# FREDZEL2020/jittor-MYC-NeRFs

Measured on AMD Instinct MI355X. Metric: ray_samples_per_sec, higher is better.
Workload: dtype f32 (emulated: 3 x f16-split MFMA products, fp32 accumulate; fp32 VALU elsewhere); 1 GPU; TensorVMSplit 300^3 (16/48 comps, MLP_Fea 150-128-128-3), 800x800 rays x 512 samples/ray (BASELINE configs[1]); ONE frame per step at every N (N>1: split over the ranks, BASELINE configs[2]), 512-ray tiles round-robin, one RCCL all_gather of [4 cap] fp32 (rgb block + depth block, written in place by the render) + two strided un-permute copies; scene=synthetic scene A (SURVEY 8d), no alpha mask, white_bg, samples_per_ray=512, rays_per_rank=640000, tile=512, chunk=640000, alpha_mask=0, emulate_world=0, arith=f32

## Files before the change

jittor-myc-nerfs_amd/csrc/tvr_march.hip:

```cpp
#include <cstdlib>
#include "tvr_device.h"
#include "tvr_kernels.h"
#include "tvr_march_body.h"
#include "tvr_gradient.h"


template <bool DENSE, bool LDSL>
__global__ __launch_bounds__(64 * MARCH_MAX_WAVES) void march_kernel(const SceneDev sc, const float *__restrict__ rays,
                                                                     const int n_rays, const int S, const int s_cap,
                                                                     const MarchSampling sm, const float eps_T,
                                                                     MarchOut mo, const tvr_dense_out dn)
{
    constexpr bool CP = false, VOL = false;
    const CpDev cp = {};
    const float *const dvol = nullptr;
#include "tvr_march_body.inc"
}

template <bool DENSE>
__global__ __launch_bounds__(64 * MARCH_VOL_WAVES, DENSE ? MARCH_VOL_OCC - 1 : MARCH_VOL_OCC) void march_vol_kernel(const SceneDev sc, const float *__restrict__ dvol, const float *__restrict__ rays,
                                                                         const int n_rays, const int S, const int s_cap, const MarchSampling sm, const float eps_T,
                                                                         MarchOut mo, const tvr_dense_out dn)
{
    constexpr bool LDSL = false, CP = false, VOL = true;
    const CpDev cp = {};
#include "tvr_march_body.inc"
}

__global__ __launch_bounds__(256) void density_volume_kernel(const SceneDev sc, float *__restrict__ out)
{
    const long long gx1 = sc.grid[0] + 1, gy1 = sc.grid[1] + 1, gz1 = sc.grid[2] + 1;
    const long long t = (long long)blockIdx.x * blockDim.x + threadIdx.x;
    if (t >= gx1 * gy1 * gz1) return;
    const long long x = t % gx1, y = (t / gx1) % gy1, z = t / (gx1 * gy1);
    const float4 *P[3] = {sc.dplane[0] + (y * gx1 + x) * 4, sc.dplane[1] + (z * gx1 + x) * 4, sc.dplane[2] + (z * gy1 + y) * 4};
    const float4 *Ln[3] = {sc.dline[0] + z * 4, sc.dline[1] + y * 4, sc.dline[2] + x * 4};
    double acc = 0.0;
#pragma unroll
    for (int i = 0; i < 3; ++i) {
#pragma unroll
        for (int g = 0; g < 4; ++g) {
            const float4 p = P[i][g], l = Ln[i][g];
            acc = acc + (double)p.x * (double)l.x;
            acc = acc + (double)p.y * (double)l.y;
            acc = acc + (double)p.z * (double)l.z;
            acc = acc + (double)p.w * (double)l.w;
        }
    }
    out[t] = (float)acc;
}

hipError_t launch_density_volume(const SceneDev &sc, float *out, hipStream_t stream)
{
    const long long n = ((long long)sc.grid[0] + 1) * ((long long)sc.grid[1] + 1) * ((long long)sc.grid[2] + 1);
    hipLaunchKernelGGL(density_volume_kernel, dim3((unsigned)((n + 255) / 256)), dim3(256), 0, stream, sc, out);
    return hipGetLastError();
}

#define COMP_LANES 8
__global__ __launch_bounds__(256) void composite_kernel(const MarchOut mo, const int n_rays, const int white_bg,
                                                        float *__restrict__ rgb_out)
{
    const int t = blockIdx.x * blockDim.x + threadIdx.x;
    const int r = t / COMP_LANES, l = t % COMP_LANES;
    const bool live = r < n_rays;
    const unsigned base = live ? mo.ray_off[r] : 0u, cnt = live ? mo.ray_cnt[r] : 0u;
    float c0 = 0.f, c1 = 0.f, c2 = 0.f;
    unsigned i = l;
    for (; i + 3 * COMP_LANES < cnt; i += 4 * COMP_LANES) {
        const float4 e0 = mo.q_out[base + i], e1 = mo.q_out[base + i + COMP_LANES], e2 = mo.q_out[base + i + 2 * COMP_LANES],
                     e3 = mo.q_out[base + i + 3 * COMP_LANES];
        c0 = c0 + e0.w * e0.x; c1 = c1 + e0.w * e0.y; c2 = c2 + e0.w * e0.z;
        c0 = c0 + e1.w * e1.x; c1 = c1 + e1.w * e1.y; c2 = c2 + e1.w * e1.z;
        c0 = c0 + e2.w * e2.x; c1 = c1 + e2.w * e2.y; c2 = c2 + e2.w * e2.z;
        c0 = c0 + e3.w * e3.x; c1 = c1 + e3.w * e3.y; c2 = c2 + e3.w * e3.z;
    }
    for (; i < cnt; i += COMP_LANES) {
        const float4 e = mo.q_out[base + i];
        c0 = c0 + e.w * e.x;
        c1 = c1 + e.w * e.y;
        c2 = c2 + e.w * e.z;
    }
#pragma unroll
    for (int off = 1; off < COMP_LANES; off <<= 1) {
        c0 = c0 + __shfl_xor(c0, off);
        c1 = c1 + __shfl_xor(c1, off);
        c2 = c2 + __shfl_xor(c2, off);
    }
    if (!live || l != 0) return;
    if (mo.counter[2] != 0u) {
        const float qnan = __int_as_float(0x7fc00000);
        rgb_out[(size_t)r * 3 + 0] = qnan; rgb_out[(size_t)r * 3 + 1] = qnan; rgb_out[(size_t)r * 3 + 2] = qnan;
        mo.depth[r] = qnan;
        return;
    }
    const float acc = mo.acc[r];
    if (white_bg) {
        const float bg = 1.0f - acc;
        c0 = c0 + bg; c1 = c1 + bg; c2 = c2 + bg;
    }
    rgb_out[(size_t)r * 3 + 0] = clamp01(c0);
    rgb_out[(size_t)r * 3 + 1] = clamp01(c1);
    rgb_out[(size_t)r * 3 + 2] = clamp01(c2);
}

__global__ __launch_bounds__(256) void scatter_rgb_kernel(const MarchOut mo, const int S, float *__restrict__ rgb_dense)
{
    const unsigned n = *mo.counter;
    for (unsigned e = blockIdx.x * blockDim.x + threadIdx.x; e < n; e += gridDim.x * blockDim.x) {
        const float4 v = mo.q_out[e];
        const size_t q = ((size_t)mo.q_ray[e] * S + mo.q_j[e]) * 3;
        rgb_dense[q] = v.x; rgb_dense[q + 1] = v.y; rgb_dense[q + 2] = v.z;
    }
}

__global__ __launch_bounds__(256) void density_feature_kernel(const SceneDev sc, const float *__restrict__ xyz, const long long m,
                                                              float *__restrict__ out)
{
    const long long t = (long long)blockIdx.x * blockDim.x + threadIdx.x;
    const long long s = t >> 2;
    const int sub = threadIdx.x & 3;
    float part = 0.0f;
    if (s < m) {
        int i0[3];
        float w[3];
#pragma unroll
        for (int k = 0; k < 3; ++k) {
            const float f = unnorm(xyz[s * 3 + k], sc.gm1[k]);
            const float fl = floorf(fminf(fmaxf(f, -2.0f), sc.gm1[k] + 2.0f));
            i0[k] = (int)fl;
            w[k] = f - fl;
        }
        const float4 a = vm_term<4, true>(sc.dplane[0], sc.dline[0], sc.grid[0], sc.grid[1], sc.grid[2], i0[0], i0[1], i0[2], w[0], w[1], w[2], sub);
        const float4 b = vm_term<4, true>(sc.dplane[1], sc.dline[1], sc.grid[0], sc.grid[2], sc.grid[1], i0[0], i0[2], i0[1], w[0], w[2], w[1], sub);
        const float4 c = vm_term<4, true>(sc.dplane[2], sc.dline[2], sc.grid[1], sc.grid[2], sc.grid[0], i0[1], i0[2], i0[0], w[1], w[2], w[0], sub);
        part = ((a.x + a.y) + (a.z + a.w)) + ((b.x + b.y) + (b.z + b.w)) + ((c.x + c.y) + (c.z + c.w));
    }
    part += __shfl_xor(part, 1);
    part += __shfl_xor(part, 2);
    if (s < m && sub == 0) out[s] = part;
}

__global__ __launch_bounds__(256) void density_gradient_kernel(const SceneDev sc, const float *__restrict__ xyz, const long long m, const float3 h, const float3 inv2h,
                                                               float *__restrict__ sigma_feature, float *__restrict__ grad)
{
    const long long t = (long long)blockIdx.x * blockDim.x + threadIdx.x;
    const long long s = t >> 2;
    const int sub = threadIdx.x & 3;
    float f[7];
#pragma unroll
    for (int j = 0; j < 7; ++j) f[j] = 0.0f;
    if (s < m) vm_grad_point(sc, xyz[s * 3], xyz[s * 3 + 1], xyz[s * 3 + 2], h, sub, f);
#pragma unroll
    for (int j = 0; j < 7; ++j) {
        f[j] += __shfl_xor(f[j], 1);
        f[j] += __shfl_xor(f[j], 2);
    }
    if (s < m && sub == 0) {
        if (sigma_feature) sigma_feature[s] = f[0];
        grad[s * 3 + 0] = (f[1] - f[2]) * inv2h.x;
        grad[s * 3 + 1] = (f[3] - f[4]) * inv2h.y;
        grad[s * 3 + 2] = (f[5] - f[6]) * inv2h.z;
    }
}

__global__ __launch_bounds__(256) void alpha_sample_kernel(const SceneDev sc, const float *__restrict__ xyz, const long long m,
                                                           float *__restrict__ out)
{
    const long long s = (long long)blockIdx.x * blockDim.x + threadIdx.x;
    if (s >= m) return;
    const float p[3] = {xyz[s * 3], xyz[s * 3 + 1], xyz[s * 3 + 2]};
    out[s] = alpha_lookup(sc, p);
}

__global__ __launch_bounds__(256) void alpha_bits_kernel(const float *__restrict__ vol, const long long n, unsigned *__restrict__ bits)
{
    const long long wd = (long long)blockIdx.x * blockDim.x + threadIdx.x;
    if (wd * 32 >= n) return;
    unsigned v = 0u;
    for (int b = 0; b < 32; ++b) {
        const long long i = wd * 32 + b;
        if (i < n && vol[i] > 0.0f) v |= 1u << b;
    }
    bits[wd] = v;
}

hipError_t launch_alpha_bits(const float *vol, long long n, unsigned *bits, hipStream_t stream)
{
    const long long words = (n + 31) / 32;
    hipLaunchKernelGGL(alpha_bits_kernel, dim3((unsigned)((words + 255) / 256)), dim3(256), 0, stream, vol, n, bits);
    return hipGetLastError();
}

template <bool DENSE, bool LDSL>
static hipError_t launch_march_t(const SceneDev &sc, const float *rays, int n_rays, int S, const MarchSampling &sm, float eps_T, const MarchOut &mo,
                                 const tvr_dense_out &dn, int waves, size_t lds, unsigned grid, hipStream_t stream)
{
    hipError_t rc = hipFuncSetAttribute((const void *)march_kernel<DENSE, LDSL>, hipFuncAttributeMaxDynamicSharedMemorySize, (int)lds);
    if (rc != hipSuccess) return rc;
    hipLaunchKernelGGL((march_kernel<DENSE, LDSL>), dim3(grid), dim3(64 * waves), lds, stream, sc, rays, n_rays, S, S, sm, eps_T, mo, dn);
    return hipGetLastError();
}

static int device_cu_count()
{
    static int cus = 0;
    if (cus == 0) {
        int dev = 0, n = 0;
        if (hipGetDevice(&dev) == hipSuccess && hipDeviceGetAttribute(&n, hipDeviceAttributeMultiprocessorCount, dev) == hipSuccess && n > 0) cus = n;
        else cus = 256;
    }
    return cus;
}

int march_cu_count() { return device_cu_count(); }

static hipError_t launch_march_vol(const SceneDev &sc, const float *dvol, const float *rays, int n_rays, int S, const MarchSampling &sm, float eps_T, const MarchOut &mo,
                                   const tvr_dense_out *dense, hipStream_t stream)
{
    const int groups = MARCH_VOL_GROUPS;
    const size_t kLds = 160 * 1024 / (size_t)groups, per_wave = (size_t)S * 6, fixed = MARCH_HDR + 64;
    int waves = (int)((kLds - fixed) / per_wave);
    waves = waves >= MARCH_VOL_WAVES ? MARCH_VOL_WAVES : (waves >= 8 ? 8 : (waves >= 4 ? 4 : (waves >= 2 ? 2 : 1)));
    const size_t lds = fixed + (size_t)waves * per_wave;
    const int n_tiles = (n_rays + MARCH_TILE - 1) / MARCH_TILE;
    long long grid = (long long)device_cu_count() * groups * (MARCH_VOL_WAVES / waves);
    if (grid > n_tiles) grid = n_tiles;
    if (grid < 1) grid = 1;
    tvr_dense_out none = {};
    const tvr_dense_out &dn = dense ? *dense : none;
    hipError_t rc = dense ? hipFuncSetAttribute((const void *)march_vol_kernel<true>, hipFuncAttributeMaxDynamicSharedMemorySize, (int)lds)
                          : hipFuncSetAttribute((const void *)march_vol_kernel<false>, hipFuncAttributeMaxDynamicSharedMemorySize, (int)lds);
    if (rc != hipSuccess) return rc;
    if (dense) hipLaunchKernelGGL((march_vol_kernel<true>), dim3((unsigned)grid), dim3(64 * waves), lds, stream, sc, dvol, rays, n_rays, S, S, sm, eps_T, mo, dn);
    else hipLaunchKernelGGL((march_vol_kernel<false>), dim3((unsigned)grid), dim3(64 * waves), lds, stream, sc, dvol, rays, n_rays, S, S, sm, eps_T, mo, dn);
    return hipGetLastError();
}

hipError_t launch_march(const SceneDev &sc, const float *rays, int n_rays, int S, const MarchSampling &sm, float eps_T,
                        const MarchOut &mo, const tvr_dense_out *dense, hipStream_t stream, const float *dvol)
{
    if (dvol) return launch_march_vol(sc, dvol, rays, n_rays, S, sm, eps_T, mo, dense, stream);
    const size_t kLds = 160 * 1024, line_bytes = ((size_t)sc.grid[0] + sc.grid[1] + sc.grid[2] + 3) * 16 * MARCH_LSTRIDE, per_wave = (size_t)S * 6;
    bool ldsl = MARCH_HDR + line_bytes + 4 * per_wave + 64 <= kLds;
    const size_t fixed = MARCH_HDR + (ldsl ? line_bytes : 0) + 64;
    int waves = (int)((kLds - fixed) / per_wave);
    waves = waves >= 16 ? 16 : (waves >= 12 ? 12 : (waves >= 8 ? 8 : (waves >= 4 ? 4 : (waves >= 2 ? 2 : 1))));
    const size_t lds = fixed + (size_t)waves * per_wave;
    const int n_tiles = (n_rays + MARCH_TILE - 1) / MARCH_TILE;
    long long grid = (long long)device_cu_count() * (16 / waves > 0 ? 16 / waves : 1);
    if (grid > n_tiles) grid = n_tiles;
    if (grid < 1) grid = 1;
    tvr_dense_out none = {};
    const tvr_dense_out &dn = dense ? *dense : none;
    if (dense) return ldsl ? launch_march_t<true, true>(sc, rays, n_rays, S, sm, eps_T, mo, dn, waves, lds, (unsigned)grid, stream)
                           : launch_march_t<true, false>(sc, rays, n_rays, S, sm, eps_T, mo, dn, waves, lds, (unsigned)grid, stream);
    return ldsl ? launch_march_t<false, true>(sc, rays, n_rays, S, sm, eps_T, mo, dn, waves, lds, (unsigned)grid, stream)
                : launch_march_t<false, false>(sc, rays, n_rays, S, sm, eps_T, mo, dn, waves, lds, (unsigned)grid, stream);
}

hipError_t launch_composite(const MarchOut &mo, int n_rays, int white_bg, float *rgb, hipStream_t stream)
{
    const long long threads = (long long)n_rays * COMP_LANES;
    hipLaunchKernelGGL(composite_kernel, dim3((unsigned)((threads + 255) / 256)), dim3(256), 0, stream, mo, n_rays, white_bg, rgb);
    return hipGetLastError();
}

hipError_t launch_scatter_rgb(const MarchOut &mo, int S, float *rgb_dense, hipStream_t stream)
{
    hipLaunchKernelGGL(scatter_rgb_kernel, dim3(1024), dim3(256), 0, stream, mo, S, rgb_dense);
    return hipGetLastError();
}

hipError_t launch_density_feature(const SceneDev &sc, const float *xyz, long long m, float *out, hipStream_t stream)
{
    const long long blocks = (m * 4 + 255) / 256;
    hipLaunchKernelGGL(density_feature_kernel, dim3((unsigned)blocks), dim3(256), 0, stream, sc, xyz, m, out);
    return hipGetLastError();
}

hipError_t launch_density_gradient(const SceneDev &sc, const float *xyz, long long m, const float h[3], const float inv2h[3], float *sigma_feature, float *grad,
                                   hipStream_t stream)
{
    const long long blocks = (m * 4 + 255) / 256;
    hipLaunchKernelGGL(density_gradient_kernel, dim3((unsigned)blocks), dim3(256), 0, stream, sc, xyz, m, make_float3(h[0], h[1], h[2]),
                       make_float3(inv2h[0], inv2h[1], inv2h[2]), sigma_feature, grad);
    return hipGetLastError();
}

hipError_t launch_alpha_sample(const SceneDev &sc, const float *xyz, long long m, float *out, hipStream_t stream)
{
    hipLaunchKernelGGL(alpha_sample_kernel, dim3((unsigned)((m + 255) / 256)), dim3(256), 0, stream, sc, xyz, m, out);
    return hipGetLastError();
}
```

jittor-myc-nerfs_amd/csrc/tvr_march_body.h:

```cpp
#pragma once
#include "tvr_device.h"
#include "tvr_kernels.h"

#define MARCH_MAX_WAVES 16
#define MARCH_TILE 16
#define MARCH_SPIN_LIMIT (1u << 22)
#define MARCH_SLOTS 64u
#ifndef MARCH_CTR_WORD
#define MARCH_CTR_WORD 1
#endif
#ifndef MARCH_TAIL
#define MARCH_TAIL 4u
#endif
#ifndef MARCH_VOL_WAVES
#define MARCH_VOL_WAVES 16
#endif
#ifndef MARCH_VOL_GROUPS
#define MARCH_VOL_GROUPS 1
#endif
#ifndef MARCH_VOL_OCC
#define MARCH_VOL_OCC 8
#endif
#define MARCH_HDR 560
#ifndef MARCH_LSTRIDE
#define MARCH_LSTRIDE 4
#endif

__device__ __forceinline__ float4 vm_term_lds(const float4 *__restrict__ P, const float4 *Ls, int W, int x0, int y0, int l0,
                                              float wx, float wy, float wl, int sub)
{
    const float ux = 1.0f - wx, uy = 1.0f - wy, ul = 1.0f - wl;
    const int Wp = W + 1;
    const unsigned cell = __umul24((unsigned)y0, (unsigned)Wp) + (unsigned)x0;
    unsigned o0 = (cell << 6) + ((unsigned)sub << 4), o1 = o0 + ((unsigned)Wp << 6);
    asm volatile("" : "+v"(o0), "+v"(o1));
    const unsigned char *pb = (const unsigned char *)P;
    const float4 t00 = *(const float4 *)(pb + (size_t)o0), t01 = *(const float4 *)(pb + (size_t)o0 + 64);
    const float4 t10 = *(const float4 *)(pb + (size_t)o1), t11 = *(const float4 *)(pb + (size_t)o1 + 64);
    const float4 *q = Ls + l0 * MARCH_LSTRIDE + sub;
    const float4 l0v = q[0], l1v = q[MARCH_LSTRIDE];
    float4 p4 = f4_mul(ux * uy, t00);
    p4 = f4_fma(wx * uy, t01, p4);
    p4 = f4_fma(ux * wy, t10, p4);
    p4 = f4_fma(wx * wy, t11, p4);
    float4 q4 = f4_mul(ul, l0v);
    q4 = f4_fma(wl, l1v, q4);
    return make_float4(p4.x * q4.x, p4.y * q4.y, p4.z * q4.z, p4.w * q4.w);
}

__device__ __forceinline__ float cp_density_quad(const SceneDev &sc, const CpDev &cp, int ix, int iy, int iz, float wx, float wy, float wz, int sub)
{
    const int tpt = cp.rd >> 2;
    const float4 *__restrict__ l0 = sc.dline[0] + (size_t)iz * tpt + sub;
    const float4 *__restrict__ l1 = sc.dline[1] + (size_t)iy * tpt + sub;
    const float4 *__restrict__ l2 = sc.dline[2] + (size_t)ix * tpt + sub;
    const float ux = 1.0f - wx, uy = 1.0f - wy, uz = 1.0f - wz;
    float part = 0.0f;
    for (int g = 0; g < tpt; g += 4) {
        const float4 a0 = l0[g], a1 = l0[g + tpt], b0 = l1[g], b1 = l1[g + tpt], c0 = l2[g], c1 = l2[g + tpt];
        const float4 a = f4_fma(wz, a1, f4_mul(uz, a0)), b = f4_fma(wy, b1, f4_mul(uy, b0)), c = f4_fma(wx, c1, f4_mul(ux, c0));
        const float tx = (a.x * b.x) * c.x, ty = (a.y * b.y) * c.y, tz = (a.z * b.z) * c.z, tw = (a.w * b.w) * c.w;
        part = part + ((tx + ty) + (tz + tw));
    }
    return part;
}

struct __attribute__((packed, aligned(4))) vol_pair { float a, b; };
__device__ __forceinline__ float vol_density(const float *__restrict__ D, int gx1, int gy1, int ix, int iy, int iz, float wx, float wy, float wz)
{
    const size_t sy = (size_t)gx1, sz = (size_t)gx1 * (size_t)gy1;
    const float *r = D + ((size_t)iz * sz + (size_t)iy * sy + (size_t)ix);
    const vol_pair p00 = *(const vol_pair *)r, p01 = *(const vol_pair *)(r + sy);
    const vol_pair p10 = *(const vol_pair *)(r + sz), p11 = *(const vol_pair *)(r + sz + sy);
    const float c00 = __builtin_fmaf(wx, p00.b - p00.a, p00.a), c01 = __builtin_fmaf(wx, p01.b - p01.a, p01.a);
    const float c10 = __builtin_fmaf(wx, p10.b - p10.a, p10.a), c11 = __builtin_fmaf(wx, p11.b - p11.a, p11.a);
    const float c0 = __builtin_fmaf(wy, c01 - c00, c00), c1 = __builtin_fmaf(wy, c11 - c10, c10);
    return __builtin_fmaf(wz, c1 - c0, c0);
}
```

jittor-myc-nerfs_amd/csrc/tvr_march_body.inc:

```
    static_assert(!(CP && LDSL), "the CP lines (up to 96 channels) do not go through LDS");
    static_assert(!(VOL && (CP || LDSL)), "the baked volume replaces the factored evaluation: no lines in LDS, no CP lines");
    extern __shared__ __attribute__((aligned(16))) unsigned char lds_raw[];
    const int lane = threadIdx.x & 63;
    const int wave = __builtin_amdgcn_readfirstlane(threadIdx.x >> 6);
    const int n_waves = blockDim.x >> 6;
    unsigned *cursor = (unsigned *)lds_raw;
    const float4 *ls0 = (const float4 *)(lds_raw + MARCH_HDR);
    const int ln0 = LDSL ? (sc.grid[2] + 1) * MARCH_LSTRIDE : 0, ln1 = LDSL ? (sc.grid[1] + 1) * MARCH_LSTRIDE : 0, ln2 = LDSL ? (sc.grid[0] + 1) * MARCH_LSTRIDE : 0;
    const float4 *ls1 = ls0 + ln0, *ls2 = ls1 + ln1;
    float *bufw = (float *)(ls2 + ln2) + (size_t)wave * s_cap;
    unsigned short *bufj = (unsigned short *)((float *)(ls2 + ln2) + (size_t)n_waves * s_cap) + (size_t)wave * s_cap;
#ifdef TVR_MARCH_TIMELINE
    unsigned long long tl_chunks = 0ull, tl_rays = 0ull;
    if (mo.stats && threadIdx.x == 0) mo.stats[32 + 8 * blockIdx.x] = __builtin_amdgcn_s_memrealtime();
#endif
    if (threadIdx.x == 0) *cursor = 0u;
    unsigned long long *slots = (unsigned long long *)(lds_raw + 16);
    if (threadIdx.x < MARCH_SLOTS) slots[threadIdx.x] = 0ull;
    unsigned long long *gstat = (unsigned long long *)(lds_raw + 16 + 8 * MARCH_SLOTS);
    if (threadIdx.x < 3) gstat[threadIdx.x] = 0ull;
    if (LDSL) {
        float4 *dst = (float4 *)(lds_raw + MARCH_HDR);
        for (int i = threadIdx.x; i < (sc.grid[2] + 1) * 4; i += blockDim.x) dst[(i >> 2) * MARCH_LSTRIDE + (i & 3)] = sc.dline[0][i];
        for (int i = threadIdx.x; i < (sc.grid[1] + 1) * 4; i += blockDim.x) dst[ln0 + (i >> 2) * MARCH_LSTRIDE + (i & 3)] = sc.dline[1][i];
        for (int i = threadIdx.x; i < (sc.grid[0] + 1) * 4; i += blockDim.x) dst[ln0 + ln1 + (i >> 2) * MARCH_LSTRIDE + (i & 3)] = sc.dline[2][i];
    }
    __syncthreads();
#ifdef TVR_MARCH_TIMELINE
    if (mo.stats && threadIdx.x == 0) mo.stats[32 + 8 * blockIdx.x + 1] = __builtin_amdgcn_s_memrealtime();
#endif
    const int sub = lane & 3;
    unsigned long long clk0 = 0ull, ref0 = 0ull;
    if (mo.stats && threadIdx.x == 0) { clk0 = __builtin_amdgcn_s_memtime(); ref0 = __builtin_amdgcn_s_memrealtime(); }

    unsigned long long st_eval = 0, st_bbox = 0, st_term = 0;
    int last_start = 0;

    for (;;) {
        unsigned ci = 0;
        if (lane == 0) ci = atomicAdd(cursor, 1u);
        ci = __builtin_amdgcn_readfirstlane(ci);
        int ray_start, ray_len;
        {
            const unsigned k = ci / MARCH_TILE, slot = k & (MARCH_SLOTS - 1u);
            if ((ci % MARCH_TILE) == 0u) {
                unsigned t = 0, len = MARCH_TILE;
                if (lane == 0) {
                    if ((long long)n_rays >= 8LL * MARCH_TILE * (long long)gridDim.x && (long long)last_start + 2LL * MARCH_TILE * (long long)gridDim.x >= (long long)n_rays)
                        len = MARCH_TAIL;
                    t = atomicAdd(mo.counter + MARCH_CTR_WORD, len);
                    const unsigned long long genw = (unsigned long long)(k + 1u) | (len == MARCH_TAIL ? 0x80000000ull : 0ull);
#ifdef TVR_FAULT_INJECT_MARCH
                    if (blockIdx.x == 0 && k == 3u) __hip_atomic_store(&slots[slot], ((unsigned long long)(k + 1u + MARCH_SLOTS) << 32) | t, __ATOMIC_RELEASE, __HIP_MEMORY_SCOPE_WORKGROUP);
                    else
#endif
                    __hip_atomic_store(&slots[slot], (genw << 32) | t, __ATOMIC_RELEASE, __HIP_MEMORY_SCOPE_WORKGROUP);
                }
                ray_start = (int)__builtin_amdgcn_readfirstlane(t);
                ray_len = (int)__builtin_amdgcn_readfirstlane(len);
            } else {
                unsigned long long v;
                unsigned spins = 0u, fault = 0u;
                for (;;) {
                    v = __hip_atomic_load(&slots[slot], __ATOMIC_ACQUIRE, __HIP_MEMORY_SCOPE_WORKGROUP);
                    const unsigned gen = (unsigned)(v >> 32) & 0x7fffffffu;
                    if (gen == k + 1u) break;
                    if (gen > k + 1u) { fault = 1u; break; }
                    if (++spins > MARCH_SPIN_LIMIT) { fault = 2u; break; }
                    __builtin_amdgcn_s_sleep(1);
                }
                if (fault) {
                    if (lane == 0) atomicOr(mo.counter + 2, fault);
                    break;
                }
                ray_start = (int)(unsigned)v;
                ray_len = (v >> 63) ? MARCH_TAIL : MARCH_TILE;
            }
        }
        if (ray_start >= n_rays) break;
        if ((int)(ci % MARCH_TILE) >= ray_len) continue;
        last_start = ray_start;
        const int ray = ray_start + (int)(ci % MARCH_TILE);
        if (ray >= n_rays) continue;
        float o[3], d[3];
#pragma unroll
        for (int k = 0; k < 3; ++k) {
            o[k] = rays[(size_t)ray * 6 + k];
            d[k] = rays[(size_t)ray * 6 + 3 + k];
        }
        const float tmin = ray_tmin(sc, o, d);
        const bool has_jit = sm.jitter != nullptr;
        const float u = has_jit ? sm.jitter[ray] : 0.0f;
        const float *__restrict__ zrow = sm.zv ? sm.zv + (size_t)ray * S : nullptr;
        float lam6 = 1.0f;
        int n6 = 0;

        float T = 1.0f, acc_l = 0.0f, dep_l = 0.0f;
        int napp = 0;
        bool seen = false, terminated = false;
        int c = 0;
        for (; c * 64 < S; ++c) {
            const int j = c * 64 + lane;
            const bool inr = j < S;
            float fj = (float)j, fj1 = (float)(j + 1);
            if (has_jit) { fj = fj + u; fj1 = fj1 + u; }
            float z = tmin + sc.step * fj;
            float z1 = tmin + sc.step * fj1;
            if (zrow) {
                z = inr ? zrow[j] : 0.0f;
                z1 = (j < S - 1) ? zrow[j + 1] : z;
            }
            float p[3], n[3], f[3];
            bool bbox = inr;
#pragma unroll
            for (int k = 0; k < 3; ++k) {
                p[k] = o[k] + d[k] * z;
                bbox = bbox & !((sc.lo[k] > p[k]) | (p[k] > sc.hi[k]));
            }
            bool valid = bbox;
            if (sc.avol != nullptr) {
                if (bbox) valid = sc.abits ? alpha_positive(sc, p) : (alpha_lookup(sc, p) > 0.0f);
            }
            int i0[3];
            float w[3];
#pragma unroll
            for (int k = 0; k < 3; ++k) {
                n[k] = (p[k] - sc.lo[k]) * sc.inv[k] - 1.0f;
                f[k] = unnorm(n[k], sc.gm1[k]);
                const float fl = floorf(f[k]);
                i0[k] = (int)fl;
                w[k] = f[k] - fl;
            }
            const unsigned long long mb = __ballot(bbox), mv = __ballot(valid);
            if (DENSE) {
                const size_t q = (size_t)ray * S + j;
                if (inr) {
                    if (dn.z) dn.z[q] = z;
                    if (dn.valid) dn.valid[q] = valid;
                    if (dn.bbox_valid) dn.bbox_valid[q] = bbox;
                    if (dn.cell) { dn.cell[q * 3] = i0[0]; dn.cell[q * 3 + 1] = i0[1]; dn.cell[q * 3 + 2] = i0[2]; }
                }
            }
            st_bbox += __popcll(mb);
            if (mv == 0ull) {
                if (DENSE && inr) {
                    const size_t q = (size_t)ray * S + j;
                    if (dn.sigma_feature) dn.sigma_feature[q] = 0.f;
                    if (dn.sigma) dn.sigma[q] = 0.f;
                    if (dn.alpha) dn.alpha[q] = 0.f;
                    if (dn.weight) dn.weight[q] = 0.f;
                }
                if (mb == 0ull && seen && !DENSE) break;
                continue;
            }
            seen = true;
            st_eval += __popcll(mv);
#ifdef TVR_MARCH_TIMELINE
            tl_chunks++;
#endif

            float sf = 0.0f;
            if constexpr (VOL) {
                if (valid) sf = vol_density(dvol, sc.grid[0] + 1, sc.grid[1] + 1, i0[0], i0[1], i0[2], w[0], w[1], w[2]);
            } else {
#pragma unroll
                for (int k4 = 0; k4 < 4; ++k4) {
                    const bool v = quad_bcast_i((int)valid, k4) != 0;
                    if (__ballot(v) == 0ull) continue;
                    const int ix = quad_bcast_i(i0[0], k4), iy = quad_bcast_i(i0[1], k4), iz = quad_bcast_i(i0[2], k4);
                    const float wx = quad_bcast_f(w[0], k4), wy = quad_bcast_f(w[1], k4), wz = quad_bcast_f(w[2], k4);
                    float part = 0.0f;
                    if constexpr (CP) {
                        if (v) part = cp_density_quad(sc, cp, ix, iy, iz, wx, wy, wz, sub);
                    } else
                    if (v && LDSL) {
                        const float4 a = vm_term_lds(sc.dplane[0], ls0, sc.grid[0], ix, iy, iz, wx, wy, wz, sub);
                        const float4 b = vm_term_lds(sc.dplane[1], ls1, sc.grid[0], ix, iz, iy, wx, wz, wy, sub);
                        const float4 cc = vm_term_lds(sc.dplane[2], ls2, sc.grid[1], iy, iz, ix, wy, wz, wx, sub);
                        part = ((a.x + a.y) + (a.z + a.w)) + ((b.x + b.y) + (b.z + b.w)) + ((cc.x + cc.y) + (cc.z + cc.w));
                    } else if (v) {
                        const float4 a = vm_term<4, false>(sc.dplane[0], sc.dline[0], sc.grid[0], sc.grid[1], sc.grid[2], ix, iy, iz, wx, wy, wz, sub);
                        const float4 b = vm_term<4, false>(sc.dplane[1], sc.dline[1], sc.grid[0], sc.grid[2], sc.grid[1], ix, iz, iy, wx, wz, wy, sub);
                        const float4 cc = vm_term<4, false>(sc.dplane[2], sc.dline[2], sc.grid[1], sc.grid[2], sc.grid[0], iy, iz, ix, wy, wz, wx, sub);
                        part = ((a.x + a.y) + (a.z + a.w)) + ((b.x + b.y) + (b.z + b.w)) + ((cc.x + cc.y) + (cc.z + cc.w));
                    }
                    part += quad_perm_f<QUAD_XOR1>(part);
                    part += quad_perm_f<QUAD_XOR2>(part);
                    if (sub == k4) sf = part;
                }
            }

            float sigma = 0.0f;
            if (valid) sigma = (sc.act == 0) ? softplus_f(sf + sc.shift) : fmaxf(sf, 0.0f);
            float dist = (j < S - 1) ? (z1 - z) : 0.0f;
            dist = dist * sc.scale;
            const float alpha = 1.0f - expf(-sigma * dist);
            const float fT = (1.0f - alpha) + 1e-10f;
            if (mo.lam6) {
                float f6 = inr ? (1.0f - alpha) + 1e-6f : 1.0f;
#pragma unroll
                for (int off = 32; off > 0; off >>= 1) f6 = f6 * __shfl_xor(f6, off);
                lam6 = lam6 * f6;
                n6 += min(64, S - c * 64);
            }
            float incl = fT;
#pragma unroll
            for (int off = 1; off < 64; off <<= 1) {
                const float t = __shfl_up(incl, off);
                if (lane >= off) incl = incl * t;
            }
            float excl = __shfl_up(incl, 1);
            if (lane == 0) excl = 1.0f;
            const float Tj = T * excl;
            const float wgt = alpha * Tj;
            acc_l += wgt;
            dep_l += wgt * z;
            const bool app = wgt > sc.thres;
            const unsigned long long ma = __ballot(app);
            if (ma) {
                const int pos = napp + __popcll(ma & ((1ull << lane) - 1ull));
                if (app) { bufw[pos] = wgt; bufj[pos] = (unsigned short)j; }
                napp += __popcll(ma);
            }
            T = T * __shfl(incl, 63);
            if (DENSE && inr) {
                const size_t q = (size_t)ray * S + j;
                if (dn.sigma_feature) dn.sigma_feature[q] = valid ? sf : 0.f;
                if (dn.sigma) dn.sigma[q] = sigma;
                if (dn.alpha) dn.alpha[q] = alpha;
                if (dn.weight) dn.weight[q] = wgt;
            }
            if (T < eps_T) { terminated = true; ++c; break; }
        }
        if (DENSE) {
            for (int cc = c; cc * 64 < S; ++cc) {
                const int j = cc * 64 + lane;
                if (j < S) {
                    const size_t q = (size_t)ray * S + j;
                    const float fjj = has_jit ? ((float)j + u) : (float)j;
                    if (dn.z) dn.z[q] = zrow ? zrow[j] : tmin + sc.step * fjj;
                    if (dn.valid) dn.valid[q] = 0;
                    if (dn.bbox_valid) dn.bbox_valid[q] = 0;
                    if (dn.cell) { dn.cell[q * 3] = 0; dn.cell[q * 3 + 1] = 0; dn.cell[q * 3 + 2] = 0; }
                    if (dn.sigma_feature) dn.sigma_feature[q] = 0.f;
                    if (dn.sigma) dn.sigma[q] = 0.f;
                    if (dn.alpha) dn.alpha[q] = 0.f;
                    if (dn.weight) dn.weight[q] = 0.f;
                }
            }
        }
        st_term += terminated ? 1 : 0;
#ifdef TVR_MARCH_TIMELINE
        tl_rays++;
#endif

        const float acc = wave_sum(acc_l);
        const float dep = wave_sum(dep_l);
        unsigned base = 0;
        if (lane == 0 && napp > 0) base = atomicAdd(mo.counter, (unsigned)napp);
        base = __shfl(base, 0);
        if (lane == 0) {
            mo.ray_off[ray] = base;
            mo.ray_cnt[ray] = (unsigned)napp;
            mo.acc[ray] = acc;
            mo.depth[ray] = dep + (1.0f - acc) * d[2];
            if (mo.lam6) mo.lam6[ray] = lam6 * expf((float)(S - n6) * 9.5367386e-7f);
            if (DENSE) {
                if (dn.bg_weight) dn.bg_weight[ray] = T;
                if (dn.acc) dn.acc[ray] = acc;
                if (dn.t_min) dn.t_min[ray] = tmin;
            }
        }
        __builtin_amdgcn_fence(__ATOMIC_ACQ_REL, "wavefront");
        for (int i = lane; i < napp; i += 64) {
            const unsigned ej = bufj[i];
            float fj = (float)ej;
            if (has_jit) fj = fj + u;
            const float z = zrow ? zrow[ej] : tmin + sc.step * fj;
            float4 qv;
            qv.x = ((o[0] + d[0] * z) - sc.lo[0]) * sc.inv[0] - 1.0f;
            qv.y = ((o[1] + d[1] * z) - sc.lo[1]) * sc.inv[1] - 1.0f;
            qv.z = ((o[2] + d[2] * z) - sc.lo[2]) * sc.inv[2] - 1.0f;
            qv.w = bufw[i];
            mo.q_pos[base + i] = qv;
            mo.q_ray[base + i] = (unsigned)ray;
            if (mo.q_j) mo.q_j[base + i] = ej;
        }
        __builtin_amdgcn_fence(__ATOMIC_ACQ_REL, "wavefront");
    }
#ifdef TVR_MARCH_TIMELINE
    if (mo.stats && lane == 0) {
        const unsigned long long te = __builtin_amdgcn_s_memrealtime();
        atomicMin((unsigned long long *)&mo.stats[32 + 8 * blockIdx.x + 2], te);
        atomicMax((unsigned long long *)&mo.stats[32 + 8 * blockIdx.x + 3], te);
        atomicAdd((unsigned long long *)&mo.stats[32 + 8 * blockIdx.x + 4], tl_chunks);
        atomicAdd((unsigned long long *)&mo.stats[32 + 8 * blockIdx.x + 5], tl_rays);
    }
#endif
    if (mo.stats) {
        if (lane == 0) {
            atomicAdd(&gstat[0], st_eval);
            atomicAdd(&gstat[1], st_bbox);
            atomicAdd(&gstat[2], st_term);
        }
        __syncthreads();
        if (threadIdx.x == 0) {
            atomicAdd((unsigned long long *)&mo.stats[TVR_STAT_SAMPLES_EVAL], gstat[0]);
            atomicAdd((unsigned long long *)&mo.stats[TVR_STAT_SAMPLES_BBOX], gstat[1]);
            atomicAdd((unsigned long long *)&mo.stats[TVR_STAT_RAYS_TERMINATED], gstat[2]);
            atomicAdd((unsigned long long *)&mo.stats[TVR_STAT_MARCH_CLK], __builtin_amdgcn_s_memtime() - clk0);
            atomicAdd((unsigned long long *)&mo.stats[TVR_STAT_MARCH_REF], __builtin_amdgcn_s_memrealtime() - ref0);
        }
    }
```

Baseline: 25.76 billion ray-samples/s.

## Add lean plain variant of volume march kernel with DPP scan and fast exp

Adds a PLAIN specialization of the density-volume march kernel, used when there are no dense outputs, alpha volume, z-values or lam6. It strips those branches and precomputes 32-bit row base pointers for the trilinear volume fetch. It also reloads rarely used kernel arguments from the kernarg segment on demand to reduce live scalar registers. For all volume kernels, it replaces the shuffle-based transmittance product scan with a DPP/permlane scan and uses hand-rolled exp/softplus. Accuracy of the custom exp/softplus and the portability of the raw kernarg offsets are the risks.

```diff
diff --git a/jittor-myc-nerfs_amd/csrc/tvr_march.hip b/jittor-myc-nerfs_amd/csrc/tvr_march.hip
--- a/jittor-myc-nerfs_amd/csrc/tvr_march.hip
+++ b/jittor-myc-nerfs_amd/csrc/tvr_march.hip
@@ -17,11 +17,12 @@
 #include "tvr_march_body.inc"
 }
 
-template <bool DENSE>
+template <bool DENSE, bool PLAIN>
 __global__ __launch_bounds__(64 * MARCH_VOL_WAVES, DENSE ? MARCH_VOL_OCC - 1 : MARCH_VOL_OCC) void march_vol_kernel(const SceneDev sc, const float *__restrict__ dvol, const float *__restrict__ rays,
                                                                          const int n_rays, const int S, const int s_cap, const MarchSampling sm, const float eps_T,
                                                                          MarchOut mo, const tvr_dense_out dn)
 {
+    static_assert(!(PLAIN && DENSE), "the plain form has no dense outputs");
     constexpr bool LDSL = false, CP = false, VOL = true;
     const CpDev cp = {};
 #include "tvr_march_body.inc"
@@ -229,11 +230,14 @@
     if (grid < 1) grid = 1;
     tvr_dense_out none = {};
     const tvr_dense_out &dn = dense ? *dense : none;
-    hipError_t rc = dense ? hipFuncSetAttribute((const void *)march_vol_kernel<true>, hipFuncAttributeMaxDynamicSharedMemorySize, (int)lds)
-                          : hipFuncSetAttribute((const void *)march_vol_kernel<false>, hipFuncAttributeMaxDynamicSharedMemorySize, (int)lds);
+    const unsigned long long vol_bytes = 4ull * (unsigned long long)(sc.grid[0] + 1) * (unsigned long long)(sc.grid[1] + 1) * (unsigned long long)(sc.grid[2] + 1);
+    const bool plain = !dense && sc.avol == nullptr && sm.zv == nullptr && mo.lam6 == nullptr && vol_bytes < (1ull << 32);
+    const void *fn = dense ? (const void *)march_vol_kernel<true, false> : (plain ? (const void *)march_vol_kernel<false, true> : (const void *)march_vol_kernel<false, false>);
+    hipError_t rc = hipFuncSetAttribute(fn, hipFuncAttributeMaxDynamicSharedMemorySize, (int)lds);
     if (rc != hipSuccess) return rc;
-    if (dense) hipLaunchKernelGGL((march_vol_kernel<true>), dim3((unsigned)grid), dim3(64 * waves), lds, stream, sc, dvol, rays, n_rays, S, S, sm, eps_T, mo, dn);
-    else hipLaunchKernelGGL((march_vol_kernel<false>), dim3((unsigned)grid), dim3(64 * waves), lds, stream, sc, dvol, rays, n_rays, S, S, sm, eps_T, mo, dn);
+    if (dense) hipLaunchKernelGGL((march_vol_kernel<true, false>), dim3((unsigned)grid), dim3(64 * waves), lds, stream, sc, dvol, rays, n_rays, S, S, sm, eps_T, mo, dn);
+    else if (plain) hipLaunchKernelGGL((march_vol_kernel<false, true>), dim3((unsigned)grid), dim3(64 * waves), lds, stream, sc, dvol, rays, n_rays, S, S, sm, eps_T, mo, dn);
+    else hipLaunchKernelGGL((march_vol_kernel<false, false>), dim3((unsigned)grid), dim3(64 * waves), lds, stream, sc, dvol, rays, n_rays, S, S, sm, eps_T, mo, dn);
     return hipGetLastError();
 }
 
diff --git a/jittor-myc-nerfs_amd/csrc/tvr_march_body.h b/jittor-myc-nerfs_amd/csrc/tvr_march_body.h
--- a/jittor-myc-nerfs_amd/csrc/tvr_march_body.h
+++ b/jittor-myc-nerfs_amd/csrc/tvr_march_body.h
@@ -77,3 +77,100 @@
     const float c0 = __builtin_fmaf(wy, c01 - c00, c00), c1 = __builtin_fmaf(wy, c11 - c10, c10);
     return __builtin_fmaf(wz, c1 - c0, c0);
 }
+
+constexpr bool PLAIN = false;
+
+struct MarchVolArgs {
+    SceneDev sc;
+    const float *dvol, *rays;
+    int n_rays, S, s_cap;
+    MarchSampling sm;
+    float eps_T;
+    MarchOut mo;
+    tvr_dense_out dn;
+};
+template <bool ON_DEMAND, typename T>
+__device__ __forceinline__ T march_arg_now(const T &arg, unsigned offset)
+{
+#if defined(__HIP_DEVICE_COMPILE__)
+    if constexpr (ON_DEMAND) {
+        const __attribute__((address_space(4))) unsigned char *ka = (const __attribute__((address_space(4))) unsigned char *)__builtin_amdgcn_kernarg_segment_ptr();
+        asm volatile("" : "+s"(ka));
+        return *(const __attribute__((address_space(4))) T *)(ka + offset);
+    }
+#endif
+    return arg;
+}
+
+__device__ __forceinline__ float vol_density32(const unsigned char *r00, const unsigned char *r01, const unsigned char *r10, const unsigned char *r11, unsigned gx1,
+                                               unsigned gy1, int ix, int iy, int iz, float wx, float wy, float wz)
+{
+    const unsigned row = __umul24((unsigned)iz, gy1) + (unsigned)iy;
+    unsigned o = (row * gx1 + (unsigned)ix) << 2;
+    asm volatile("" : "+v"(o));
+    const vol_pair p00 = *(const vol_pair *)(r00 + (size_t)o), p01 = *(const vol_pair *)(r01 + (size_t)o);
+    const vol_pair p10 = *(const vol_pair *)(r10 + (size_t)o), p11 = *(const vol_pair *)(r11 + (size_t)o);
+    const float c00 = __builtin_fmaf(wx, p00.b - p00.a, p00.a), c01 = __builtin_fmaf(wx, p01.b - p01.a, p01.a);
+    const float c10 = __builtin_fmaf(wx, p10.b - p10.a, p10.a), c11 = __builtin_fmaf(wx, p11.b - p11.a, p11.a);
+    const float c0 = __builtin_fmaf(wy, c01 - c00, c00), c1 = __builtin_fmaf(wy, c11 - c10, c10);
+    return __builtin_fmaf(wz, c1 - c0, c0);
+}
+
+#ifndef MARCH_VOL_LEAN
+#define MARCH_VOL_LEAN 1
+#endif
+__device__ __forceinline__ float march_expf(float x)
+{
+    const float p = x * 0x1.715476p+0f;
+    const float r = __builtin_rintf(p);
+    float lo = __builtin_fmaf(x, 0x1.715476p+0f, -p);
+    lo = __builtin_fmaf(x, 0x1.4ae0bep-26f, lo);
+    return __builtin_ldexpf(__builtin_amdgcn_exp2f((p - r) + lo), (int)r);
+}
+__device__ __forceinline__ float march_softplus(float x)
+{
+    if (x > 20.0f) return x;
+    const float t = march_expf(x);
+    const float u = 1.0f + t, d = u - 1.0f;
+    const float rc = __builtin_amdgcn_rcpf(d);
+    float q = t * rc;
+    q = __builtin_fmaf(__builtin_fmaf(-d, q, t), rc, q);
+    const float lg = __builtin_amdgcn_logf(u) * 0x1.62e430p-1f;
+    return d == 0.0f ? t : lg * q;
+}
+
+#define MARCH_DPP_WAVE_SHR1 0x138
+#define MARCH_DPP_SAME 0xE4
+template <int CTRL, int ROWS>
+__device__ __forceinline__ float march_dpp_mov(float old, float v)
+{
+    return __int_as_float(__builtin_amdgcn_update_dpp(__float_as_int(old), __float_as_int(v), CTRL, ROWS, 0xF, false));
+}
+template <int N>
+__device__ __forceinline__ float march_up(float v)
+{
+    float t = march_dpp_mov<MARCH_DPP_WAVE_SHR1, 0xF>(1.0f, v);
+#pragma unroll
+    for (int i = 1; i < N; ++i) t = march_dpp_mov<MARCH_DPP_WAVE_SHR1, 0xF>(t, t);
+    return t;
+}
+__device__ __forceinline__ void scan_mul_dpp(float &x, float &excl, float &last)
+{
+    x = x * march_up<1>(x);
+    x = x * march_up<2>(x);
+    x = x * march_up<4>(x);
+    x = x * march_up<8>(x);
+    {
+        const auto q = __builtin_amdgcn_permlane16_swap(__float_as_uint(x), __float_as_uint(x), false, false);
+        const auto s = __builtin_amdgcn_permlane32_swap(q[0], q[1], false, false);
+        float t = march_dpp_mov<MARCH_DPP_SAME, 0x6>(1.0f, __uint_as_float(s[0]));
+        t = march_dpp_mov<MARCH_DPP_SAME, 0x8>(t, __uint_as_float(q[0]));
+        x = x * t;
+    }
+    {
+        const auto h = __builtin_amdgcn_permlane32_swap(__float_as_uint(x), __float_as_uint(x), false, false);
+        x = x * march_dpp_mov<MARCH_DPP_SAME, 0xC>(1.0f, __uint_as_float(h[0]));
+    }
+    excl = march_up<1>(x);
+    last = __int_as_float(__builtin_amdgcn_readlane(__float_as_int(x), 63));
+}
diff --git a/jittor-myc-nerfs_amd/csrc/tvr_march_body.inc b/jittor-myc-nerfs_amd/csrc/tvr_march_body.inc
--- a/jittor-myc-nerfs_amd/csrc/tvr_march_body.inc
+++ b/jittor-myc-nerfs_amd/csrc/tvr_march_body.inc
@@ -30,8 +30,13 @@
     if (mo.stats && threadIdx.x == 0) mo.stats[32 + 8 * blockIdx.x + 1] = __builtin_amdgcn_s_memrealtime();
 #endif
     const int sub = lane & 3;
+    const unsigned char *vrow[4] = {nullptr, nullptr, nullptr, nullptr};
+    if constexpr (PLAIN) {
+        const size_t vsy = (size_t)(sc.grid[0] + 1) * 4, vsz = vsy * (size_t)(sc.grid[1] + 1);
+        vrow[0] = (const unsigned char *)dvol; vrow[1] = vrow[0] + vsy; vrow[2] = vrow[0] + vsz; vrow[3] = vrow[2] + vsy;
+    }
     unsigned long long clk0 = 0ull, ref0 = 0ull;
-    if (mo.stats && threadIdx.x == 0) { clk0 = __builtin_amdgcn_s_memtime(); ref0 = __builtin_amdgcn_s_memrealtime(); }
+    if (march_arg_now<PLAIN>(mo.stats, offsetof(MarchVolArgs, mo.stats)) && threadIdx.x == 0) { clk0 = __builtin_amdgcn_s_memtime(); ref0 = __builtin_amdgcn_s_memrealtime(); }
 
     unsigned long long st_eval = 0, st_bbox = 0, st_term = 0;
     int last_start = 0;
@@ -48,7 +53,7 @@
                 if (lane == 0) {
                     if ((long long)n_rays >= 8LL * MARCH_TILE * (long long)gridDim.x && (long long)last_start + 2LL * MARCH_TILE * (long long)gridDim.x >= (long long)n_rays)
                         len = MARCH_TAIL;
-                    t = atomicAdd(mo.counter + MARCH_CTR_WORD, len);
+                    t = atomicAdd(march_arg_now<PLAIN>(mo.counter, offsetof(MarchVolArgs, mo.counter)) + MARCH_CTR_WORD, len);
                     const unsigned long long genw = (unsigned long long)(k + 1u) | (len == MARCH_TAIL ? 0x80000000ull : 0ull);
 #ifdef TVR_FAULT_INJECT_MARCH
                     if (blockIdx.x == 0 && k == 3u) __hip_atomic_store(&slots[slot], ((unsigned long long)(k + 1u + MARCH_SLOTS) << 32) | t, __ATOMIC_RELEASE, __HIP_MEMORY_SCOPE_WORKGROUP);
@@ -70,7 +75,7 @@
                     __builtin_amdgcn_s_sleep(1);
                 }
                 if (fault) {
-                    if (lane == 0) atomicOr(mo.counter + 2, fault);
+                    if (lane == 0) atomicOr(march_arg_now<PLAIN>(mo.counter, offsetof(MarchVolArgs, mo.counter)) + 2, fault);
                     break;
                 }
                 ray_start = (int)(unsigned)v;
@@ -82,16 +87,18 @@
         last_start = ray_start;
         const int ray = ray_start + (int)(ci % MARCH_TILE);
         if (ray >= n_rays) continue;
+        const float *__restrict__ const rays_r = march_arg_now<PLAIN>(rays, offsetof(MarchVolArgs, rays));
+        const float *const jit_r = march_arg_now<PLAIN>(sm.jitter, offsetof(MarchVolArgs, sm.jitter));
         float o[3], d[3];
 #pragma unroll
         for (int k = 0; k < 3; ++k) {
-            o[k] = rays[(size_t)ray * 6 + k];
-            d[k] = rays[(size_t)ray * 6 + 3 + k];
+            o[k] = rays_r[(size_t)ray * 6 + k];
+            d[k] = rays_r[(size_t)ray * 6 + 3 + k];
         }
         const float tmin = ray_tmin(sc, o, d);
-        const bool has_jit = sm.jitter != nullptr;
-        const float u = has_jit ? sm.jitter[ray] : 0.0f;
-        const float *__restrict__ zrow = sm.zv ? sm.zv + (size_t)ray * S : nullptr;
+        const bool has_jit = jit_r != nullptr;
+        const float u = has_jit ? jit_r[ray] : 0.0f;
+        const float *__restrict__ zrow = (!PLAIN && sm.zv) ? sm.zv + (size_t)ray * S : nullptr;
         float lam6 = 1.0f;
         int n6 = 0;
 
@@ -118,7 +125,7 @@
                 bbox = bbox & !((sc.lo[k] > p[k]) | (p[k] > sc.hi[k]));
             }
             bool valid = bbox;
-            if (sc.avol != nullptr) {
+            if (!PLAIN && sc.avol != nullptr) {
                 if (bbox) valid = sc.abits ? alpha_positive(sc, p) : (alpha_lookup(sc, p) > 0.0f);
             }
             int i0[3];
@@ -131,6 +138,7 @@
                 i0[k] = (int)fl;
                 w[k] = f[k] - fl;
             }
+            if constexpr (PLAIN) asm volatile("" : "+v"(i0[0]), "+v"(i0[1]), "+v"(i0[2]), "+v"(w[0]), "+v"(w[1]), "+v"(w[2]));
             const unsigned long long mb = __ballot(bbox), mv = __ballot(valid);
             if (DENSE) {
                 const size_t q = (size_t)ray * S + j;
@@ -161,6 +169,9 @@
 
             float sf = 0.0f;
             if constexpr (VOL) {
+                if constexpr (PLAIN) {
+                    if (valid) sf = vol_density32(vrow[0], vrow[1], vrow[2], vrow[3], (unsigned)(sc.grid[0] + 1), (unsigned)(sc.grid[1] + 1), i0[0], i0[1], i0[2], w[0], w[1], w[2]);
+                } else
                 if (valid) sf = vol_density(dvol, sc.grid[0] + 1, sc.grid[1] + 1, i0[0], i0[1], i0[2], w[0], w[1], w[2]);
             } else {
 #pragma unroll
@@ -191,26 +202,34 @@
             }
 
             float sigma = 0.0f;
+            constexpr bool LEAN = VOL && MARCH_VOL_LEAN;
+            if constexpr (LEAN) {
+                if (valid) sigma = (sc.act == 0) ? march_softplus(sf + sc.shift) : fmaxf(sf, 0.0f);
+            } else
             if (valid) sigma = (sc.act == 0) ? softplus_f(sf + sc.shift) : fmaxf(sf, 0.0f);
             float dist = (j < S - 1) ? (z1 - z) : 0.0f;
             dist = dist * sc.scale;
-            const float alpha = 1.0f - expf(-sigma * dist);
+            const float alpha = 1.0f - (LEAN ? march_expf(-sigma * dist) : expf(-sigma * dist));
             const float fT = (1.0f - alpha) + 1e-10f;
-            if (mo.lam6) {
+            if (!PLAIN && mo.lam6) {
                 float f6 = inr ? (1.0f - alpha) + 1e-6f : 1.0f;
 #pragma unroll
                 for (int off = 32; off > 0; off >>= 1) f6 = f6 * __shfl_xor(f6, off);
                 lam6 = lam6 * f6;
                 n6 += min(64, S - c * 64);
             }
-            float incl = fT;
-#pragma unroll
-            for (int off = 1; off < 64; off <<= 1) {
-                const float t = __shfl_up(incl, off);
-                if (lane >= off) incl = incl * t;
-            }
-            float excl = __shfl_up(incl, 1);
-            if (lane == 0) excl = 1.0f;
+            float incl = fT, excl, last;
+            if constexpr (VOL) {
+                scan_mul_dpp(incl, excl, last);
+            } else {
+#pragma unroll
+                for (int off = 1; off < 64; off <<= 1) {
+                    const float t = __shfl_up(incl, off);
+                    if (lane >= off) incl = incl * t;
+                }
+                excl = __shfl_up(incl, 1);
+                if (lane == 0) excl = 1.0f;
+            }
             const float Tj = T * excl;
             const float wgt = alpha * Tj;
             acc_l += wgt;
@@ -222,7 +241,8 @@
                 if (app) { bufw[pos] = wgt; bufj[pos] = (unsigned short)j; }
                 napp += __popcll(ma);
             }
-            T = T * __shfl(incl, 63);
+            if constexpr (VOL) T = T * last;
+            else T = T * __shfl(incl, 63);
             if (DENSE && inr) {
                 const size_t q = (size_t)ray * S + j;
                 if (dn.sigma_feature) dn.sigma_feature[q] = valid ? sf : 0.f;
@@ -256,15 +276,16 @@
 
         const float acc = wave_sum(acc_l);
         const float dep = wave_sum(dep_l);
+        const MarchOut mt = march_arg_now<PLAIN>(mo, offsetof(MarchVolArgs, mo));
         unsigned base = 0;
-        if (lane == 0 && napp > 0) base = atomicAdd(mo.counter, (unsigned)napp);
+        if (lane == 0 && napp > 0) base = atomicAdd(mt.counter, (unsigned)napp);
         base = __shfl(base, 0);
         if (lane == 0) {
-            mo.ray_off[ray] = base;
-            mo.ray_cnt[ray] = (unsigned)napp;
-            mo.acc[ray] = acc;
-            mo.depth[ray] = dep + (1.0f - acc) * d[2];
-            if (mo.lam6) mo.lam6[ray] = lam6 * expf((float)(S - n6) * 9.5367386e-7f);
+            mt.ray_off[ray] = base;
+            mt.ray_cnt[ray] = (unsigned)napp;
+            mt.acc[ray] = acc;
+            mt.depth[ray] = dep + (1.0f - acc) * d[2];
+            if (!PLAIN && mt.lam6) mt.lam6[ray] = lam6 * expf((float)(S - n6) * 9.5367386e-7f);
             if (DENSE) {
                 if (dn.bg_weight) dn.bg_weight[ray] = T;
                 if (dn.acc) dn.acc[ray] = acc;
@@ -282,9 +303,9 @@
             qv.y = ((o[1] + d[1] * z) - sc.lo[1]) * sc.inv[1] - 1.0f;
             qv.z = ((o[2] + d[2] * z) - sc.lo[2]) * sc.inv[2] - 1.0f;
             qv.w = bufw[i];
-            mo.q_pos[base + i] = qv;
-            mo.q_ray[base + i] = (unsigned)ray;
-            if (mo.q_j) mo.q_j[base + i] = ej;
+            mt.q_pos[base + i] = qv;
+            mt.q_ray[base + i] = (unsigned)ray;
+            if (mt.q_j) mt.q_j[base + i] = ej;
         }
         __builtin_amdgcn_fence(__ATOMIC_ACQ_REL, "wavefront");
     }
@@ -297,7 +318,8 @@
         atomicAdd((unsigned long long *)&mo.stats[32 + 8 * blockIdx.x + 5], tl_rays);
     }
 #endif
-    if (mo.stats) {
+    unsigned long long *const stats_r = march_arg_now<PLAIN>(mo.stats, offsetof(MarchVolArgs, mo.stats));
+    if (stats_r) {
         if (lane == 0) {
             atomicAdd(&gstat[0], st_eval);
             atomicAdd(&gstat[1], st_bbox);
@@ -305,10 +327,10 @@
         }
         __syncthreads();
         if (threadIdx.x == 0) {
-            atomicAdd((unsigned long long *)&mo.stats[TVR_STAT_SAMPLES_EVAL], gstat[0]);
-            atomicAdd((unsigned long long *)&mo.stats[TVR_STAT_SAMPLES_BBOX], gstat[1]);
-            atomicAdd((unsigned long long *)&mo.stats[TVR_STAT_RAYS_TERMINATED], gstat[2]);
-            atomicAdd((unsigned long long *)&mo.stats[TVR_STAT_MARCH_CLK], __builtin_amdgcn_s_memtime() - clk0);
-            atomicAdd((unsigned long long *)&mo.stats[TVR_STAT_MARCH_REF], __builtin_amdgcn_s_memrealtime() - ref0);
-        }
-    }
+            atomicAdd((unsigned long long *)&stats_r[TVR_STAT_SAMPLES_EVAL], gstat[0]);
+            atomicAdd((unsigned long long *)&stats_r[TVR_STAT_SAMPLES_BBOX], gstat[1]);
+            atomicAdd((unsigned long long *)&stats_r[TVR_STAT_RAYS_TERMINATED], gstat[2]);
+            atomicAdd((unsigned long long *)&stats_r[TVR_STAT_MARCH_CLK], __builtin_amdgcn_s_memtime() - clk0);
+            atomicAdd((unsigned long long *)&stats_r[TVR_STAT_MARCH_REF], __builtin_amdgcn_s_memrealtime() - ref0);
+        }
+    }
```

Result: faster. 26.09 billion ray-samples/s (median of 6 runs) (+1.3%).
